# synsense/HaghighatshoarMuir2024

Measured on AMD Instinct MI355X. Metric: audio samples/sec through STHT+RZCC+SNN beamform, 7-mic 48kHz 360-DoA; DoA MAE vs ref, higher is better.
Workload: dtype f64

## Files before the change

### haghighatshoarmuir2024_amd/csrc/api.hip

```cpp
#include <math.h>
#include <string.h>

#include <new>
#include <vector>

#include "micloc_internal.h"

using namespace micloc;

static thread_local int g_last_hip = 0;

static int hip_failed(hipError_t e)
{
    g_last_hip = (int)e;
    (void)hipGetLastError();
    return MICLOC_ERR_HIP;
}

#define HIP_TRY(expr)                                \
    do {                                             \
        hipError_t _e = (expr);                      \
        if (_e != hipSuccess) return hip_failed(_e); \
    } while (0)

// ... 65 lines not shown
{
    int ct = (C + 15) / 16;
    if (ct > 4 && ct <= 8) ct = 8;
    return ct;
}

struct FrontOffsets {
    size_t h, pre, scratch, spikes;
};

struct WsLayout : FrontOffsets {
    size_t partial, total;
};

WsLayout ws_layout(const micloc_plan *p, int B, int T)
{
    WsLayout w{};
    const size_t Ts = (size_t)micloc_padded_T(T);
    const size_t planar = align256((size_t)B * p->C * Ts * sizeof(double));
    int Gp = p->W.GT > 0 ? 16 * p->W.GT : 16;
    size_t off = 0;
    w.h = off;
    off += planar;
    w.pre = off;
    off += planar;
    w.scratch = off;
    off += rzcc_scratch_bytes(B * p->C, T, p->robust_width, p->chunk_frames);
    w.spikes = off;
    off += align256((size_t)B * T * p->C);
    w.partial = off;
    {
        const size_t pb = beamform_partial_bytes(B, T, Gp);
        const int ct = pad_ct(p->C);
        const size_t pc = ct <= 8 ? cov_partial_bytes(B, T, ct) : 0;
        off += pb > pc ? pb : pc;
    }
    w.total = off;
    return w;
}

bool bad_batch(int B) { return B < 1 || B > 65535; }

bool bad_ws(const void *ws, size_t have, size_t need)
{
    return ws == nullptr || have < need || (reinterpret_cast<uintptr_t>(ws) & 255) != 0;
}

double *ws_doubles(void *ws, size_t offset) { return reinterpret_cast<double *>(static_cast<unsigned char *>(ws) + offset); }

int gen_chunk_frames(int CT)
{
    for (int c = 256; c <= 4096; c += 256)
        if (beamform_nchunks_ct(c, CT) == 1 && beamform_nchunks_ct(c + 1, CT) == 2) return c;
    return 0;
}

int window_quantum(const micloc_plan *p)
{
    if (!p->W_is_complex) return lif_beamform_chunk_frames(p->W, p->ntab);
    if (p->W.CT == 1 && (p->W.GT & 1) == 0) return 256;
    return gen_chunk_frames(p->W.CT);
}

int window_args(int T, int window, int hop, int quantum, int B, int *nW)
{
    if (T < 1 || quantum < 1) return MICLOC_ERR_INVALID;
    if (window < 1 || hop < 1 || window % quantum != 0 || hop % quantum != 0) return MICLOC_ERR_SHAPE;
    const long long n = window_count(T, window, hop);
    if (n * (long long)B > 0x7fffffffll) return MICLOC_ERR_SHAPE;
    *nW = (int)n;
    return MICLOC_OK;
}

int window_readout(const micloc_plan *p, const double *partial, int B, int T, int nch, int quantum, int window, int hop, double *power_w,
                   int32_t *argmax_w, double *power, int32_t *argmax, hipStream_t st)
{
    if (nch != (T + quantum - 1) / quantum) return MICLOC_ERR_INVALID;
    const int Gp = 16 * p->W.GT, cp = p->W_is_complex ? 1 : 0;
    HIP_TRY(launch_window_power(partial, B, T, nch, Gp, p->G_out, cp, cp ? Gp / 2 : 0, quantum, window, hop, power_w, argmax_w, st));
    if (power || argmax) HIP_TRY(launch_power_argmax(partial, B, T, nch, Gp, p->G_out, cp, cp ? Gp / 2 : 0, power, argmax, st));
    return MICLOC_OK;
}

hipError_t lif_beamform_oneshot(const BeamformW &W, const NeuronTab &nt, const int8_t *spikes, int B, int T, double *y, double *partial,
                                hipStream_t stream, int *nchunks)
{
    hipError_t e = hipSuccess;
    if (launch_lif_beamform_lean(W, nt, spikes, B, T, y, partial, stream, nchunks, &e)) return e;
    return launch_lif_beamform(W, nt, spikes, B, T, y, partial, stream, nchunks);
}

int plan_kind(const micloc_plan *p, bool cpx)
{
    if (!p->d_W || (!cpx && !p->d_ntab)) return MICLOC_ERR_NOT_SET;
    return (p->W_is_complex != 0) == cpx ? MICLOC_OK : MICLOC_ERR_SHAPE;
}

int window_check(const micloc_plan *p, bool cpx, int B, int T, int window, int hop)
{
    int rc = plan_kind(p, cpx), nW = 0;
    if (rc != MICLOC_OK) return rc;
    const int q = window_quantum(p);
    rc = window_args(T, window, hop, q, B, &nW);
    return rc == MICLOC_OK ? q : rc;
}

int cov_check(const micloc_plan *p, bool want_power)
{
    if (!p->d_ntab) return MICLOC_ERR_NOT_SET;
    if (want_power && (!p->d_W || p->W_is_complex)) return p->d_W ? MICLOC_ERR_SHAPE : MICLOC_ERR_NOT_SET;
    return pad_ct(p->C) > 8 ? MICLOC_ERR_SHAPE : MICLOC_OK;
}

struct Front {
    int rc;
    const void *src;
    int Ts;
};

Front front_end(const micloc_plan *p, bool cpx, const double *x, int B, int T, void *ws, const FrontOffsets &o, int8_t *spikes, int stages,
                hipStream_t st)
{
    Front f{MICLOC_OK, nullptr, micloc_padded_T(T)};
    double *h = ws_doubles(ws, o.h);
    hipError_t e = (stages & MICLOC_STAGE_STHT) ? launch_stht(p->taps, x, h, B, T, p->M, f.Ts, st, false) : hipSuccess;
    if (cpx) {
        double *pre = ws_doubles(ws, o.pre);
        f.src = pre;
        if (e == hipSuccess)
            e = launch_bandpass_rzcc(p->iir, h, B * p->C, p->C, T, f.Ts, p->robust_width, p->bipolar, pre, nullptr, nullptr, st, x, p->M,
                                     p->taps.shift);
    } else {
        int8_t *spk = spikes ? spikes : static_cast<int8_t *>(ws) + o.spikes;
        f.src = spk;
        const int phases = (stages & MICLOC_STAGE_ENCODE) ? RZ_PHASE_ALL
                                                          : ((stages & MICLOC_STAGE_ENCODE_SCAN) ? RZ_PHASE_SCAN : 0) |
                                                                ((stages & MICLOC_STAGE_ENCODE_REST) ? RZ_PHASE_ENCODE : 0);
        if (e == hipSuccess && phases)
            e = launch_bandpass_rzcc(p->iir, h, B * p->C, p->C, T, f.Ts, p->robust_width, p->bipolar, nullptr, spk,
                                     static_cast<char *>(ws) + o.scratch, st, x, p->M, p->taps.shift, p->chunk_frames, phases);
    }
    if (e != hipSuccess) f.rc = hip_failed(e);
    return f;
}

int power_tail(const micloc_plan *p, const void *src, int B, int T, int Ts, double *y, double *power, int32_t *argmax, double *partial,
               hipStream_t st)
{
    const int Gp = 16 * p->W.GT, cpx = p->W_is_complex ? 1 : 0;
    if (!power && !argmax) partial = nullptr;
    int nch = 0;
    if (cpx)
        HIP_TRY(launch_planar_beamform(p->W, static_cast<const double *>(src), B, T, Ts, y, 1, partial, st, &nch));
    else
        HIP_TRY(lif_beamform_oneshot(p->W, p->ntab, static_cast<const int8_t *>(src), B, T, y, partial, st, &nch));
    if (partial) HIP_TRY(launch_power_argmax(partial, B, T, nch, Gp, p->G_out, cpx, cpx ? Gp / 2 : 0, power, argmax, st));
    return MICLOC_OK;
}

int window_tail(const micloc_plan *p, const void *src, int B, int T, int Ts, int quantum, int window, int hop, double *power_w,
                int32_t *argmax_w, double *power, int32_t *argmax, double *partial, hipStream_t st)
{
    int nch = 0;
    if (p->W_is_complex)
        HIP_TRY(launch_planar_beamform(p->W, static_cast<const double *>(src), B, T, Ts, nullptr, 1, partial, st, &nch));
    else
        HIP_TRY(launch_lif_beamform(p->W, p->ntab, static_cast<const int8_t *>(src), B, T, nullptr, partial, st, &nch));
    return window_readout(p, partial, B, T, nch, quantum, window, hop, power_w, argmax_w, power, argmax, st);
}

int cov_tail(const micloc_plan *p, const int8_t *spikes, int B, int T, int t_start, double *cov, double *power, int32_t *argmax, double *partial,
             hipStream_t st)
{
    const int CT = pad_ct(p->C);
    const bool want_power = power || argmax;
    HIP_TRY(launch_lif_cov(p->ntab, spikes, B, T, p->C, CT, t_start, partial, st));
    HIP_TRY(launch_cov_power(partial, B, T, CT, p->C, T - t_start, want_power ? p->W.Wp : nullptr, want_power ? 16 * p->W.GT : 16,
                             want_power ? p->G_out : 0, cov, power, argmax, st));
    return MICLOC_OK;
}

}

extern "C" {

int micloc_abi_version(void) { return MICLOC_ABI_VERSION; }

int micloc_last_hip_error(void) { return g_last_hip; }

const char *micloc_status_string(int status)
{
    switch (status) {
        case MICLOC_OK: return "ok";
        case MICLOC_ERR_INVALID: return "invalid argument";
        case MICLOC_ERR_SHAPE: return "shape mismatch";
        case MICLOC_ERR_WORKSPACE: return "workspace too small or misaligned (256-byte alignment required)";
        case MICLOC_ERR_NOT_SET: return "neuron kernel or beamforming matrix not set on the plan";
        case MICLOC_ERR_HIP: return "HIP runtime error (see micloc_last_hip_error)";
        case MICLOC_ERR_NO_DEVICE: return "no usable HIP device";
        default: return "unknown status";
    }
}

int micloc_padded_T(int T) { return T <= 0 ? 8 : (T + 7) & ~7; }

int micloc_plan_create(const micloc_config *cfg, micloc_plan **out)
{
    if (!cfg || !out) return MICLOC_ERR_INVALID;
    *out = nullptr;
    if (cfg->num_mic <= 0 || cfg->stht_len <= 0 || !cfg->stht_kernel) return MICLOC_ERR_INVALID;
    if (cfg->iir_len < 1 || cfg->iir_len > MICLOC_MAX_IIR || !cfg->iir_b || !cfg->iir_a) return MICLOC_ERR_INVALID;
    if (cfg->iir_a[0] == 0.0 || cfg->robust_width < 1) return MICLOC_ERR_INVALID;
    int ndev = 0;
    if (hipGetDeviceCount(&ndev) != hipSuccess || ndev <= 0 || cfg->device < 0 || cfg->device >= ndev)
        return MICLOC_ERR_NO_DEVICE;
    {
        hipDeviceProp_t prop;
        if (hipGetDeviceProperties(&prop, cfg->device) != hipSuccess || strncmp(prop.gcnArchName, "gfx950", 6) != 0)
            return MICLOC_ERR_NO_DEVICE;
    }

    micloc_plan *p = new (std::nothrow) micloc_plan();
// ... 138 lines not shown
            Wp[(size_t)(M + m) * Gp + g] = wi;
            Wp[(size_t)m * Gp + Ghp + g] = -wi;
            Wp[(size_t)(M + m) * Gp + Ghp + g] = wr;
        }
    return set_W(p, Wp, CT, Gp / 16, C, 2 * G, 1, G);
}

int micloc_plan_generation(const micloc_plan *p) { return p ? p->generation : -1; }

int micloc_stream_create_cu_range(int device, int cu_lo, int cu_hi, void **stream)
{
    if (!stream || device < 0) return MICLOC_ERR_INVALID;
    *stream = nullptr;
    DeviceGuard guard(device);
    hipDeviceProp_t prop;
    HIP_TRY(hipGetDeviceProperties(&prop, device));
    if (strncmp(prop.gcnArchName, "gfx950", 6) != 0) return MICLOC_ERR_INVALID;
    constexpr int NXCD = 8;
    const int ncu = prop.multiProcessorCount;
    if (ncu != 256) return MICLOC_ERR_INVALID;
    const int per = ncu / NXCD;
    if (cu_lo < 0 || cu_hi > per || cu_lo >= cu_hi) return MICLOC_ERR_INVALID;
    std::vector<uint32_t> mask((size_t)(ncu + 31) / 32, 0u);
    for (int c = cu_lo; c < cu_hi; ++c)
        for (int x = 0; x < NXCD; ++x) {
            const int bit = c * NXCD + x;
            mask[bit / 32] |= 1u << (bit % 32);
        }
    hipStream_t st = nullptr;
    HIP_TRY(hipExtStreamCreateWithCUMask(&st, (uint32_t)mask.size(), mask.data()));
    *stream = st;
    return MICLOC_OK;
}

int micloc_stream_destroy(void *stream)
{
    if (!stream) return MICLOC_ERR_INVALID;
    HIP_TRY(hipStreamDestroy((hipStream_t)stream));
    return MICLOC_OK;
}

int micloc_plan_set_encoder_chunk(micloc_plan *p, int chunk_frames)
{
    if (!p) return MICLOC_ERR_INVALID;
    p->chunk_frames = chunk_frames;
    return MICLOC_OK;
}

int micloc_plan_encoder_chunks(const micloc_plan *p, int B, int T)
{
    if (!p || bad_batch(B) || T < 1) return MICLOC_ERR_INVALID;
    return rzcc_chunks(B * p->C, T, p->robust_width, p->chunk_frames);
}

size_t micloc_workspace_bytes(const micloc_plan *p, int B, int T)
{
    if (!p || bad_batch(B) || T < 1) return 0;
    return ws_layout(p, B, T).total;
}

size_t micloc_lif_beamform_workspace_bytes(const micloc_plan *p, int B, int T)
{
    if (!p || bad_batch(B) || T < 1 || p->W.GT < 1) return 0;
    return align256(beamform_partial_bytes(B, T, 16 * p->W.GT));
}

int micloc_stht_f64(const micloc_plan *p, const double *x, int B, int T, double *h, int Ts, void *stream)
{
    if (!p || !x || !h || bad_batch(B) || T < 1) return MICLOC_ERR_INVALID;
    DeviceGuard guard(p->device);
    if (Ts != micloc_padded_T(T)) return MICLOC_ERR_SHAPE;
    HIP_TRY(launch_stht(p->taps, x, h, B, T, p->M, Ts, (hipStream_t)stream));
    return MICLOC_OK;
}

int micloc_bandpass_rzcc_f64(const micloc_plan *p, const double *h, int B, int T, int Ts, double *pre,
                             int8_t *spikes, void *ws, size_t ws_bytes, void *stream)
{
    if (!p || !h || bad_batch(B) || T < 1 || (!pre && !spikes)) return MICLOC_ERR_INVALID;
    DeviceGuard guard(p->device);
    if (Ts != micloc_padded_T(T)) return MICLOC_ERR_SHAPE;
    const int nl = B * p->C;
    if (spikes && bad_ws(ws, ws_bytes, rzcc_scratch_bytes(nl, T, p->robust_width, p->chunk_frames))) return MICLOC_ERR_WORKSPACE;
    HIP_TRY(launch_bandpass_rzcc(p->iir, h, nl, p->C, T, Ts, p->robust_width, p->bipolar, pre, spikes, ws,
                                 (hipStream_t)stream, nullptr, 0, 0, p->chunk_frames));
    return MICLOC_OK;
}

int micloc_lif_beamform_f64(const micloc_plan *p, const int8_t *spikes, int B, int T, double *y, double *power,
                            int32_t *argmax, void *ws, size_t ws_bytes, void *stream)
{
    if (!p || !spikes || bad_batch(B) || T < 1 || (!y && !power && !argmax)) return MICLOC_ERR_INVALID;
    DeviceGuard guard(p->device);
    const int rc = plan_kind(p, false);
    if (rc != MICLOC_OK) return rc;
    if ((power || argmax) && bad_ws(ws, ws_bytes, beamform_partial_bytes(B, T, 16 * p->W.GT))) return MICLOC_ERR_WORKSPACE;
    return power_tail(p, spikes, B, T, 0, y, power, argmax, ws_doubles(ws, 0), (hipStream_t)stream);
}

int micloc_beamform_c128_f64(const micloc_plan *p, const double *pre, int B, int T, int Ts, double *y, double *power,
                             int32_t *argmax, void *ws, size_t ws_bytes, void *stream)
{
    if (!p || !pre || bad_batch(B) || T < 1 || (!y && !power && !argmax)) return MICLOC_ERR_INVALID;
    DeviceGuard guard(p->device);
    if (Ts != micloc_padded_T(T)) return MICLOC_ERR_SHAPE;
    const int rc = plan_kind(p, true);
    if (rc != MICLOC_OK) return rc;
    if ((power || argmax) && bad_ws(ws, ws_bytes, beamform_partial_bytes(B, T, 16 * p->W.GT))) return MICLOC_ERR_WORKSPACE;
    return power_tail(p, pre, B, T, Ts, y, power, argmax, ws_doubles(ws, 0), (hipStream_t)stream);
}

int micloc_snn_pipeline_f64(const micloc_plan *p, const double *x, int B, int T, int8_t *spikes, double *y,
                            double *power, int32_t *argmax, void *ws, size_t ws_bytes, void *stream)
{
    return micloc_snn_pipeline_stages_f64(p, x, B, T, spikes, y, power, argmax, ws, ws_bytes, stream, MICLOC_STAGE_ALL);
}

int micloc_snn_pipeline_stages_f64(const micloc_plan *p, const double *x, int B, int T, int8_t *spikes, double *y,
                                   double *power, int32_t *argmax, void *ws, size_t ws_bytes, void *stream, int stages)
{
    if (!p || !x || bad_batch(B) || T < 1 || (!spikes && !y && !power && !argmax)) return MICLOC_ERR_INVALID;
    DeviceGuard guard(p->device);
    if (stages <= 0 || (stages & ~(MICLOC_STAGE_ALL | MICLOC_STAGE_ENCODE_SCAN | MICLOC_STAGE_ENCODE_REST))) return MICLOC_ERR_INVALID;
    const bool want_bf = y || power || argmax;
    const int rc = want_bf ? plan_kind(p, false) : MICLOC_OK;
    if (rc != MICLOC_OK) return rc;
    const WsLayout w = ws_layout(p, B, T);
    if (bad_ws(ws, ws_bytes, w.total)) return MICLOC_ERR_WORKSPACE;
    const Front f = front_end(p, false, x, B, T, ws, w, spikes, stages, (hipStream_t)stream);
    if (f.rc != MICLOC_OK) return f.rc;
    if (!want_bf || !(stages & MICLOC_STAGE_BEAMFORM)) return MICLOC_OK;
    return power_tail(p, f.src, B, T, f.Ts, y, power, argmax, ws_doubles(ws, w.partial), (hipStream_t)stream);
}

int micloc_beamformer_pipeline_f64(const micloc_plan *p, const double *x, int B, int T, double *y, double *power,
                                   int32_t *argmax, void *ws, size_t ws_bytes, void *stream)
{
    if (!p || !x || bad_batch(B) || T < 1 || (!y && !power && !argmax)) return MICLOC_ERR_INVALID;
    DeviceGuard guard(p->device);
    const int rc = plan_kind(p, true);
    if (rc != MICLOC_OK) return rc;
    const WsLayout w = ws_layout(p, B, T);
    if (bad_ws(ws, ws_bytes, w.total)) return MICLOC_ERR_WORKSPACE;
    const Front f = front_end(p, true, x, B, T, ws, w, nullptr, MICLOC_STAGE_ALL, (hipStream_t)stream);
    if (f.rc != MICLOC_OK) return f.rc;
    return power_tail(p, f.src, B, T, f.Ts, y, power, argmax, ws_doubles(ws, w.partial), (hipStream_t)stream);
}

int micloc_window_quantum(const micloc_plan *p)
{
    if (!p) return MICLOC_ERR_INVALID;
    if (plan_kind(p, p->W_is_complex) != MICLOC_OK) return MICLOC_ERR_NOT_SET;
    const int q = window_quantum(p);
    return q > 0 ? q : MICLOC_ERR_INVALID;
}

int micloc_window_count(int T, int window, int hop, int quantum)
{
    int nW = 0;
    const int rc = window_args(T, window, hop, quantum, 1, &nW);
    return rc == MICLOC_OK ? nW : rc;
}

size_t micloc_window_workspace_bytes(const micloc_plan *p, int B, int T, int window, int hop, int pipeline)
{
    if (!p || bad_batch(B) || T < 1 || micloc_window_quantum(p) < 1) return 0;
    int nW = 0;
    if (window_args(T, window, hop, window_quantum(p), B, &nW) != MICLOC_OK) return 0;
// ... 1219 lines not shown
```

### haghighatshoarmuir2024_amd/csrc/micloc_internal.h

```cpp
#pragma once
#include <hip/hip_runtime.h>
#include <stddef.h>
#include <stdint.h>

#include "../../include/micloc_hip.h"

namespace micloc {

constexpr bool VARIANT_WS_FOUR_KSTEPS = false;
constexpr bool VARIANT_STHT_VECTOR_FORM = false;
constexpr bool VARIANT_STHT_WIDE_TWO_TILES = false;
constexpr bool VARIANT_STHT_ONE_TILE = false;
constexpr bool VARIANT_WS_GENERAL_ONLY = false;

__device__ __forceinline__ int xcd_walk(int L, int n)
{
    const int per = n >> 3;
    return L < 8 * per ? (L & 7) * per + (L >> 3) : L;
}

constexpr int STHT_R = 8;
constexpr int STHT_TILE = 64 * STHT_R;
constexpr int STHT_MAX_MB = 8;

struct SthtTaps {
    const double *taps;
    int ngroups;
    int klo;
    int kstep;
    int halo;
    int shift;
};

hipError_t launch_stht(const SthtTaps &tp, const double *x, double *h, int B, int T, int M, int Ts,
                       hipStream_t stream, bool write_re = true);
size_t stht_lds_bytes(const SthtTaps &tp, int M);

struct IirCoef {
    double b[MICLOC_MAX_IIR];
    double a[MICLOC_MAX_IIR];
    int n;
};

size_t rzcc_scratch_bytes(int nlanes, int T, int robust_width, int chunk_frames);
int rzcc_chunks(int nlanes, int T, int robust_width, int chunk_frames);
constexpr int RZ_PHASE_SCAN = 1, RZ_PHASE_ENCODE = 2, RZ_PHASE_ALL = 3;
hipError_t launch_bandpass_rzcc(const IirCoef &coef, const double *h, int nlanes, int C, int T, int Ts,
                                int robust_width, int bipolar, double *pre, int8_t *spikes, void *scratch,
                                hipStream_t stream, const double *xin = nullptr, int M = 0, int shift = 0,
                                int chunk_frames = 0, int phases = RZ_PHASE_ALL);
size_t rzcc_stream_state_bytes(int nlanes);
hipError_t launch_stream_encode(const IirCoef &coef, const double *h, int nlanes, int C, int T, int Ts, int robust_width,
                                int bipolar, int8_t *spikes, int Ttot, long long t_base, int first_tile, int final_tile,
                                void *state, hipStream_t stream, int pos_lo = 0, const int *clk = nullptr);
hipError_t launch_stream_horizon(const void *enc_state, int nlanes, int bipolar, int t_end, int final_, int chunk_frames, int base_chunk,
                                 int nwin, int *ctl, hipStream_t stream, int clocked = 0);
constexpr int STREAM_CLK_T = 16;
constexpr int STREAM_CLK_BASE = 17;
constexpr int STREAM_CLK_SHIFT = 18;
constexpr int STREAM_CLK_TEND = 19;
hipError_t launch_stream_begin_tile(int *ctl, int8_t *win, int8_t *tmp, int B, size_t row_bytes, int C, int n, int cap, int chunk_frames,
                                    hipStream_t stream);
hipError_t launch_stream_tick(int *ctl, hipStream_t stream);
hipError_t launch_stht_wrap_rows(double *h, const double *wrap, int B, int M, int Ts, int col0, int n, int half, const int *ctl,
                                 hipStream_t stream);
hipError_t launch_stream_commit(int *ctl, int block_chunks, hipStream_t stream);
hipError_t launch_stream_accumulate(const double *partial, int B, int nwin, int Gp, int G, const int *range, const int *ctl,
                                    double *acc, const int *frames_ptr, double *power, int32_t *argmax, hipStream_t stream);
constexpr int STREAM_BLOCK_CHUNKS = 32;
hipError_t launch_zero_fill(void *ptr, size_t bytes, hipStream_t stream);
hipError_t launch_pack_planar(const double *src, double *dst, int B, int T, int C, int Ts, hipStream_t stream);
hipError_t launch_unpack_planar(const double *src, double *dst, int B, int T, int C, int Ts, hipStream_t stream);

constexpr int BF_WAVES = 8;
constexpr int BF_NT = 4;
constexpr int BF_CHUNK = BF_WAVES * BF_NT * 16;

struct BeamformW {
    const double *Wp;
    int CT, GT;
    int C, G;
    int complex_pairs;
    const int *chunk_range = nullptr;
};

struct NeuronTab {
    const double *tab;
    int n;
    int NK;
};

size_t beamform_partial_bytes(int B, int T, int Gp);
hipError_t launch_lif_beamform(const BeamformW &W, const NeuronTab &nt, const int8_t *spikes, int B, int T,
                               double *y, double *partial, hipStream_t stream, int *nchunks);
bool launch_lif_beamform_lean(const BeamformW &W, const NeuronTab &nt, const int8_t *spikes, int B, int T, double *y, double *partial,
                              hipStream_t stream, int *nchunks, hipError_t *err);
hipError_t launch_planar_beamform(const BeamformW &W, const double *pre, int B, int T, int Ts, double *y,
                                  int y_complex, double *partial, hipStream_t stream, int *nchunks);
hipError_t launch_power_argmax(const double *partial, int B, int T, int nchunks, int Gp, int G, int complex_pairs,
                               int Ghalf_pad, double *power, int32_t *argmax, hipStream_t stream);
int beamform_nchunks(int T);
int beamform_nchunks_ct(int T, int CT);
int lif_beamform_chunk_frames(const BeamformW &W, const NeuronTab &nt);

long long window_count(int T, int window, int hop);
hipError_t launch_window_power(const double *partial, int B, int T, int nchunks, int Gp, int G, int complex_pairs, int Ghalf_pad,
                               int chunk_frames, int window, int hop, double *power_w, int32_t *argmax_w, hipStream_t stream);

int stream_window_slots(int window, int hop);
size_t stream_window_state_bytes(int B, int G, int window, int hop);
hipError_t launch_stream_windows(const double *partial, int B, int nwin, int Gp, int G, int complex_pairs, int Ghp, int chunk_frames,
                                 const int *ctl, int final_tile, int window, int hop, int max_windows, void *win_state, double *power_w,
                                 int32_t *argmax_w, double *latest_power, int32_t *latest_argmax, hipStream_t stream);

struct StreamComplexLayout {
    size_t z, carry, acc, total;
};
StreamComplexLayout stream_complex_layout(int B, int C, int G, int iir_n, int CH);
int stream_complex_chunks(int max_tile, int CH);
hipError_t launch_stream_complex_bandpass(const IirCoef &co, const double *h, int nl, int n, size_t row_stride, double *staging, int S,
                                          int CH, void *state, const StreamComplexLayout &L, hipStream_t stream);
hipError_t launch_stream_complex_accumulate(const double *partial, int B, int Ks, int Gp, int G, int CH, int final_tile, void *state,
                                            const StreamComplexLayout &L, double *power, int32_t *argmax, hipStream_t stream);
hipError_t launch_stream_complex_slide(const double *staging, int nl, int S, int CH, void *state, const StreamComplexLayout &L,
                                       hipStream_t stream);

hipError_t launch_lif_beamform_f32(const BeamformW &W, const NeuronTab &nt, const int8_t *spikes, int B, int T,
                                   double *partial, hipStream_t stream, int *nchunks);

size_t cov_partial_bytes(int B, int T, int CT);
hipError_t launch_lif_cov(const NeuronTab &nt, const int8_t *spikes, int B, int T, int C, int CT, int t_start,
                          double *partial, hipStream_t stream);
hipError_t launch_cov_power(const double *partial, int B, int T, int CT, int C, int Tn, const double *Wp, int Gp, int G,
// ... 111 lines not shown
```

Before: 3.727 billion.

## Add warp-specialized single-pass RZCC sweep kernel with fallback for overflowing lanes

Adds a new bandpass+RZCC spike encoder that uses dedicated loader waves, an IIR/cumsum wave and a zero-crossing/cluster-resolve wave. They run in a triple-buffered LDS pipeline, one block per 64 lanes. Lanes whose ring overflows are flagged and reprocessed by a per-lane fallback kernel. The path is used when the filter order is 5, the encode phase is requested and a single chunk covers T; otherwise the old launcher runs. It aims to cut the multi-pass scan/encode cost but adds a zero-fill pass and a fallback launch, with complex correctness conditions.

New measurement: 3.864 billion (median of 6 runs). 3.7% higher.

```diff
diff --git a/haghighatshoarmuir2024_amd/csrc/api.hip b/haghighatshoarmuir2024_amd/csrc/api.hip
--- a/haghighatshoarmuir2024_amd/csrc/api.hip
+++ b/haghighatshoarmuir2024_amd/csrc/api.hip
@@ -171,6 +171,18 @@
     return MICLOC_OK;
 }
 
+static hipError_t bandpass_rzcc_spikes(const IirCoef &coef, const double *h, int nlanes, int C, int T, int Ts, int robust_width, int bipolar,
+                                       int8_t *spikes, void *scratch, hipStream_t stream, const double *xin, int M, int shift,
+                                       int chunk_frames, int phases)
+{
+    hipError_t e = hipSuccess;
+    if (launch_bandpass_rzcc_sweep(coef, h, nlanes, C, T, Ts, robust_width, bipolar, spikes, scratch, stream, xin, M, shift, chunk_frames,
+                                   phases, &e))
+        return e;
+    return launch_bandpass_rzcc(coef, h, nlanes, C, T, Ts, robust_width, bipolar, nullptr, spikes, scratch, stream, xin, M, shift,
+                                chunk_frames, phases);
+}
+
 hipError_t lif_beamform_oneshot(const BeamformW &W, const NeuronTab &nt, const int8_t *spikes, int B, int T, double *y, double *partial,
                                 hipStream_t stream, int *nchunks)
 {
@@ -226,7 +238,7 @@
                                                           : ((stages & MICLOC_STAGE_ENCODE_SCAN) ? RZ_PHASE_SCAN : 0) |
                                                                 ((stages & MICLOC_STAGE_ENCODE_REST) ? RZ_PHASE_ENCODE : 0);
         if (e == hipSuccess && phases)
-            e = launch_bandpass_rzcc(p->iir, h, B * p->C, p->C, T, f.Ts, p->robust_width, p->bipolar, nullptr, spk,
+            e = bandpass_rzcc_spikes(p->iir, h, B * p->C, p->C, T, f.Ts, p->robust_width, p->bipolar, spk,
                                      static_cast<char *>(ws) + o.scratch, st, x, p->M, p->taps.shift, p->chunk_frames, phases);
     }
     if (e != hipSuccess) f.rc = hip_failed(e);
@@ -531,8 +543,12 @@
     if (Ts != micloc_padded_T(T)) return MICLOC_ERR_SHAPE;
     const int nl = B * p->C;
     if (spikes && bad_ws(ws, ws_bytes, rzcc_scratch_bytes(nl, T, p->robust_width, p->chunk_frames))) return MICLOC_ERR_WORKSPACE;
-    HIP_TRY(launch_bandpass_rzcc(p->iir, h, nl, p->C, T, Ts, p->robust_width, p->bipolar, pre, spikes, ws,
-                                 (hipStream_t)stream, nullptr, 0, 0, p->chunk_frames));
+    if (spikes && !pre)
+        HIP_TRY(bandpass_rzcc_spikes(p->iir, h, nl, p->C, T, Ts, p->robust_width, p->bipolar, spikes, ws, (hipStream_t)stream, nullptr, 0, 0,
+                                     p->chunk_frames, RZ_PHASE_ALL));
+    else
+        HIP_TRY(launch_bandpass_rzcc(p->iir, h, nl, p->C, T, Ts, p->robust_width, p->bipolar, pre, spikes, ws,
+                                     (hipStream_t)stream, nullptr, 0, 0, p->chunk_frames));
     return MICLOC_OK;
 }
 
diff --git a/haghighatshoarmuir2024_amd/csrc/micloc_internal.h b/haghighatshoarmuir2024_amd/csrc/micloc_internal.h
--- a/haghighatshoarmuir2024_amd/csrc/micloc_internal.h
+++ b/haghighatshoarmuir2024_amd/csrc/micloc_internal.h
@@ -12,6 +12,7 @@
 constexpr bool VARIANT_STHT_WIDE_TWO_TILES = false;
 constexpr bool VARIANT_STHT_ONE_TILE = false;
 constexpr bool VARIANT_WS_GENERAL_ONLY = false;
+constexpr bool VARIANT_RZ_TWO_SLOTS = false;
 
 __device__ __forceinline__ int xcd_walk(int L, int n)
 {
@@ -49,6 +50,9 @@
                                 int robust_width, int bipolar, double *pre, int8_t *spikes, void *scratch,
                                 hipStream_t stream, const double *xin = nullptr, int M = 0, int shift = 0,
                                 int chunk_frames = 0, int phases = RZ_PHASE_ALL);
+bool launch_bandpass_rzcc_sweep(const IirCoef &coef, const double *h, int nlanes, int C, int T, int Ts, int robust_width, int bipolar,
+                                int8_t *spikes, void *scratch, hipStream_t stream, const double *xin, int M, int shift, int chunk_frames,
+                                int phases, hipError_t *err);
 size_t rzcc_stream_state_bytes(int nlanes);
 hipError_t launch_stream_encode(const IirCoef &coef, const double *h, int nlanes, int C, int T, int Ts, int robust_width,
                                 int bipolar, int8_t *spikes, int Ttot, long long t_base, int first_tile, int final_tile,
diff --git a/haghighatshoarmuir2024_amd/csrc/rzcc_sweep.hip b/haghighatshoarmuir2024_amd/csrc/rzcc_sweep.hip
--- /dev/null
+++ b/haghighatshoarmuir2024_amd/csrc/rzcc_sweep.hip
@@ -0,0 +1,758 @@
+#include "micloc_internal.h"
+
+#include <type_traits>
+
+#pragma clang diagnostic ignored "-Wpass-failed"
+
+namespace micloc {
+namespace rzsweep {
+
+constexpr int RZ_RING_SWEEP = 32;
+
+template <int N>
+struct Iir {
+    double z[N > 1 ? N - 1 : 1];
+
+    __device__ __forceinline__ void init()
+    {
+#pragma unroll
+        for (int i = 0; i < (N > 1 ? N - 1 : 1); ++i) z[i] = 0.0;
+    }
+
+    __device__ __forceinline__ double step(const IirCoef &coef, double xin)
+    {
+        double y;
+        if (N == 1) {
+            y = __builtin_fma(coef.b[0], xin, 0.0);
+        } else {
+            y = __builtin_fma(coef.b[0], xin, z[0]);
+#pragma unroll
+            for (int i = 0; i < N - 2; ++i)
+                z[i] = __builtin_fma(-coef.a[i + 1], y, __builtin_fma(coef.b[i + 1], xin, z[i + 1]));
+            z[N - 2] = __builtin_fma(-coef.a[N - 1], y, coef.b[N - 1] * xin);
+        }
+        return y;
+    }
+};
+
+template <int N>
+__device__ __forceinline__ void pin_coef(const IirCoef &coef)
+{
+#pragma unroll
+    for (int i = 0; i < N; ++i) asm volatile("; filter coefficient resident" ::"s"(coef.b[i]), "s"(coef.a[i]));
+}
+
+template <int W, typename WordAt, typename ValAt, typename Emit>
+__device__ __forceinline__ void resolve_cluster_regs(int s, int stride, int count, int w, Emit emit, WordAt word_at, ValAt val_at,
+                                                     double sgn)
+{
+    int P[W];
+    double V[W];
+#pragma unroll
+    for (int u = 0; u < W; ++u) {
+        const int kc = u < count ? s + u * stride : s;
+        P[u] = *word_at(kc) >> 1;
+        V[u] = *val_at(kc) * sgn;
+    }
+    unsigned alive = (1u << count) - 1u;
+    while (alive) {
+        int best = -1, pb = 0;
+        double bv = 0.0;
+#pragma unroll
+        for (int u = 0; u < W; ++u) {
+            if (((alive >> u) & 1u) && (best < 0 || V[u] >= bv)) {
+                best = u;
+                bv = V[u];
+                pb = P[u];
+            }
+        }
+        emit(pb);
+        alive &= ~(1u << best);
+#pragma unroll
+        for (int u = 0; u < W; ++u) {
+            const int d = P[u] - pb;
+            if ((d < 0 ? -d : d) < w) alive &= ~(1u << u);
+        }
+    }
+}
+
+template <int MAXW = 16, typename WordAt, typename ValAt, typename Emit>
+__device__ __forceinline__ void resolve_cluster(int s, int e, int stride, int w, Emit emit, WordAt word_at, ValAt val_at,
+                                                double sgn)
+{
+    int remaining = (e - s + stride - 1) / stride;
+    if (remaining <= 4) {
+        resolve_cluster_regs<4>(s, stride, remaining, w, emit, word_at, val_at, sgn);
+        return;
+    }
+    if (remaining <= 8) {
+        resolve_cluster_regs<8>(s, stride, remaining, w, emit, word_at, val_at, sgn);
+        return;
+    }
+    if (MAXW >= 16 && remaining <= 16) {
+        resolve_cluster_regs<16>(s, stride, remaining, w, emit, word_at, val_at, sgn);
+        return;
+    }
+    while (remaining > 0) {
+        int best = -1;
+        double bv = 0.0;
+        for (int k = s; k < e; k += 4 * stride) {
+            int wk[4];
+            double vk[4];
+#pragma unroll
+            for (int u = 0; u < 4; ++u) {
+                const int kk = k + u * stride;
+                const int kc = kk < e ? kk : s;
+                wk[u] = *word_at(kc);
+                vk[u] = *val_at(kc) * sgn;
+            }
+#pragma unroll
+            for (int u = 0; u < 4; ++u) {
+                const int kk = k + u * stride;
+                if (kk < e && wk[u] >= 0 && (best < 0 || vk[u] >= bv)) {
+                    best = kk;
+                    bv = vk[u];
+                }
+            }
+        }
+        const int wb = *word_at(best);
+        const int pb = wb >> 1;
+        emit(pb);
+        *word_at(best) = ~wb;
+        --remaining;
+        for (int k = best - stride; k >= s; k -= stride) {
+            const int wk = *word_at(k);
+            const int pk = (wk < 0 ? ~wk : wk) >> 1;
+            if (pb - pk >= w) break;
+            if (wk >= 0) {
+                *word_at(k) = ~wk;
+                --remaining;
+            }
+        }
+        for (int k = best + stride; k < e; k += stride) {
+            const int wk = *word_at(k);
+            const int pk = (wk < 0 ? ~wk : wk) >> 1;
+            if (pk - pb >= w) break;
+            if (wk >= 0) {
+                *word_at(k) = ~wk;
+                --remaining;
+            }
+        }
+    }
+}
+
+constexpr int RZ_MT = 16;
+
+__device__ __forceinline__ void rise_fall_step(unsigned &r, unsigned &f, double a, double b)
+{
+    asm("v_cmp_gt_f64 vcc, %2, %3\n\tv_addc_co_u32_e32 %0, vcc, %0, %0, vcc\n\tv_cmp_lt_f64 vcc, %2, %3\n\tv_addc_co_u32_e32 %1, vcc, %1, %1, vcc"
+        : "+v"(r), "+v"(f)
+        : "v"(a), "v"(b)
+        : "vcc");
+}
+
+struct RzGeom {
+    int P;
+    int Lt;
+    int Vt;
+    int V2t;
+};
+
+struct RzSpan {
+    int m_lo, m_hi;
+    int own_lo, own_hi;
+    bool at_end;
+};
+
+__host__ __device__ inline RzSpan rz_span(const RzGeom &g, int p, int NM)
+{
+    RzSpan s;
+    s.m_lo = p == 0 ? 0 : p * g.Lt - g.Vt;
+    const int hi = (p + 1) * g.Lt + g.V2t;
+    s.m_hi = (p == g.P - 1 || hi > NM) ? NM : hi;
+    s.own_lo = p == 0 ? 0 : p * g.Lt * RZ_MT;
+    s.own_hi = p == g.P - 1 ? 0x7fffffff : (p + 1) * g.Lt * RZ_MT;
+    s.at_end = s.m_hi == NM;
+    return s;
+}
+
+constexpr int RZ_DIR_RISE = 1, RZ_DIR_FALL = 2, RZ_DIR_UNKNOWN = 3;
+
+template <int PHASE, typename XT>
+__device__ __forceinline__ void rz_loader_np(XT &X, const double *__restrict__ h, const double *__restrict__ xin, int base,
+                                             int nlanes, int C, int T, int Ts, int M, int shift, int NMc, int nstep, int lane,
+                                             unsigned long long *tab)
+{
+    constexpr int NP = 2;
+    constexpr int phase = PHASE;
+    const int tl = lane & 15;
+    const int sq = lane >> 4;
+    constexpr int NJ = 16;
+    double v[2][NJ];
+    {
+        int g = base + lane;
+        g = g < nlanes ? g : nlanes - 1;
+        const int bb = g / C, cc = g - bb * C;
+        const bool r = xin != nullptr && cc < M;
+        const double *b0 = r ? xin + (size_t)bb * T * M + cc : h + (size_t)g * Ts;
+        tab[lane] = (unsigned long long)(size_t)b0 | (r ? 1ull : 0ull);
+        __builtin_amdgcn_fence(__ATOMIC_RELEASE, "wavefront");
+        __builtin_amdgcn_wave_barrier();
+        __builtin_amdgcn_fence(__ATOMIC_ACQUIRE, "wavefront");
+    }
+    const int sh = shift % T;
+    auto issue_loads = [&](int q, auto set) {
+        constexpr int S = decltype(set)::value;
+        int mm = phase + NP * q;
+        mm = mm < NMc ? mm : NMc - 1;
+        const int t = mm * RZ_MT + tl;
+        const int tc = t < Ts ? t : Ts - 1;
+        int tr = (t < T ? t : T - 1) - sh;
+        tr = tr < 0 ? tr + T : tr;
+        const unsigned i_roll = (unsigned)tr * (unsigned)M, i_lin = (unsigned)tc;
+        {
+            const unsigned ta = (unsigned)(size_t)(&tab[sq]);
+            typedef __attribute__((address_space(1))) double gdouble;
+#pragma unroll
+            for (int j0 = 0; j0 < NJ; j0 += 4) {
+                unsigned long long e[4];
+#pragma unroll
+                for (int u = 0; u < 4; ++u)
+                    asm volatile("ds_read_b64 %0, %1 offset:%2" : "=v"(e[u]) : "v"(ta), "n"((j0 + u) * 32));
+                asm volatile("s_waitcnt lgkmcnt(0)" : "+v"(e[0]), "+v"(e[1]), "+v"(e[2]), "+v"(e[3]));
+#pragma unroll
+                for (int u = 0; u < 4; ++u)
+                    v[S][j0 + u] = reinterpret_cast<const gdouble *>((size_t)(e[u] & ~7ull))[(e[u] & 1ull) ? i_roll : i_lin];
+            }
+        }
+    };
+    auto write_tile = [&](int buf, auto set) {
+        constexpr int S = decltype(set)::value;
+        {
+            const unsigned wa = (unsigned)(size_t)(&X[buf][tl][sq]);
+#pragma unroll
+            for (int j = 0; j < NJ; ++j) {
+                const double vj = v[S][j];
+                asm volatile("ds_write_b64 %0, %1 offset:%2" ::"v"(wa), "v"(vj), "n"(j * 32));
+            }
+        }
+    };
+    using set0 = std::integral_constant<int, 0>;
+    using set1 = std::integral_constant<int, 1>;
+    issue_loads(0, set0{});
+    issue_loads(1, set1{});
+    if (phase == 0) {
+        write_tile(0, set0{});
+        issue_loads(2, set0{});
+    }
+    __syncthreads();
+    auto iter = [&](int k, auto pos, auto set) {
+        constexpr int I = decltype(pos)::value;
+        if constexpr (((I + 1) % NP) == phase) {
+            const int m = k + 1;
+            write_tile(m % 3, set);
+            issue_loads((m - phase) / NP + 2, set);
+        }
+        __syncthreads();
+    };
+    using p0 = std::integral_constant<int, 0>;
+    using p1 = std::integral_constant<int, 1>;
+    using p2 = std::integral_constant<int, 2>;
+    using p3 = std::integral_constant<int, 3>;
+    int k = 0;
+    for (; k + 3 < nstep; k += 4) {
+        iter(k, p0{}, set0{});
+        iter(k + 1, p1{}, set1{});
+        iter(k + 2, p2{}, set1{});
+        iter(k + 3, p3{}, set0{});
+    }
+    if (k < nstep) iter(k++, p0{}, set0{});
+    if (k < nstep) iter(k++, p1{}, set1{});
+    if (k < nstep) iter(k++, p2{}, set1{});
+}
+
+template <int N, int RING>
+__global__ __launch_bounds__(384, 5) void bandpass_rzcc_sweep_kernel(const double *__restrict__ h, int8_t *__restrict__ spikes,
+                                                                     int *__restrict__ flag_count, int *__restrict__ flag_list,
+                                                                     IirCoef coef, int nlanes, int C, int T, int Ts, int w, int bipolar,
+                                                                     const double *__restrict__ xin, int M, int shift)
+{
+    constexpr int SW = 64;
+    constexpr int ROW = SW + 1;
+    __shared__ __attribute__((aligned(16))) double X[3][RZ_MT][ROW];
+    __shared__ double ringV[RING][SW];
+    __shared__ int ringP[RING][SW];
+    __shared__ int nPub[SW];
+    __shared__ int polPub[SW];
+    __shared__ int deadPub[SW];
+    __shared__ int ovPub[SW];
+    __shared__ int oldPub[2][SW];
+    __shared__ unsigned long long ldTab[SW];
+
+    const int wave_hw = threadIdx.x >> 6;
+    const int wave = wave_hw == 0 ? 0 : wave_hw - 1;
+    const int lane = threadIdx.x & 63;
+    const int base = xcd_walk(blockIdx.x, gridDim.x) * SW;
+    const int NM = (T + RZ_MT - 1) / RZ_MT;
+    const int NSTEP = NM + 2;
+    const int lane_g = base + lane;
+    const bool active = lane_g < nlanes;
+    const int lane_c = active ? lane_g : nlanes - 1;
+
+    if (wave_hw == 0) {
+        rz_loader_np<0>(X, h, xin, base, nlanes, C, T, Ts, M, shift, NM, NSTEP, lane, ldTab);
+        return;
+    }
+    if (wave_hw == 1) {
+        rz_loader_np<1>(X, h, xin, base, nlanes, C, T, Ts, M, shift, NM, NSTEP, lane, ldTab);
+        return;
+    }
+
+    if (wave == 1) {
+        Iir<N> iir;
+        iir.init();
+        double cs = 0.0;
+        pin_coef<N>(coef);
+        __syncthreads();
+        for (int k = 0; k < NSTEP; ++k) {
+            if (k < NM) {
+                const int buf = k % 3;
+                const int tb = k * RZ_MT;
+                const int steps = (T - tb) < RZ_MT ? (T - tb) : RZ_MT;
+                if (steps == RZ_MT) {
+                    double xr[RZ_MT];
+                    const unsigned addr = (unsigned)(size_t)(&X[buf][0][lane]);
+#pragma unroll
+                    for (int j = 0; j < RZ_MT; ++j)
+                        asm volatile("ds_read_b64 %0, %1 offset:%2" : "=v"(xr[j]) : "v"(addr), "n"(j * ROW * 8));
+                    asm volatile("s_waitcnt lgkmcnt(0)"
+                                 : "+v"(xr[0]), "+v"(xr[1]), "+v"(xr[2]), "+v"(xr[3]), "+v"(xr[4]), "+v"(xr[5]), "+v"(xr[6]), "+v"(xr[7]),
+                                   "+v"(xr[8]), "+v"(xr[9]), "+v"(xr[10]), "+v"(xr[11]), "+v"(xr[12]), "+v"(xr[13]), "+v"(xr[14]),
+                                   "+v"(xr[15]));
+#pragma unroll
+                    for (int j = 0; j < RZ_MT; ++j) {
+                        cs = cs + iir.step(coef, xr[j]);
+                        xr[j] = cs;
+                    }
+#pragma unroll
+                    for (int j = 0; j < RZ_MT; ++j) X[buf][j][lane] = xr[j];
+                } else {
+                    for (int j = 0; j < steps; ++j) {
+                        cs = cs + iir.step(coef, X[buf][j][lane]);
+                        X[buf][j][lane] = cs;
+                    }
+                }
+            }
+            __syncthreads();
+        }
+        return;
+    }
+
+    if (wave == 2) {
+        double prev = __builtin_nan("");
+        int left = 0;
+        int n = 0;
+        int dir = 0;
+        int ffall = 0;
+        bool livel = true;
+        nPub[lane] = 0;
+        polPub[lane] = 0;
+        ovPub[lane] = 0;
+        __syncthreads();
+        for (int k = 0; k < NSTEP; ++k) {
+            if (k >= 1 && k <= NM) {
+                const int m = k - 1;
+                const int tbase = m * RZ_MT;
+                const int steps = (T - tbase) < RZ_MT ? (T - tbase) : RZ_MT;
+                const int o0 = oldPub[0][lane], o1 = oldPub[1][lane];
+                const int oldest = bipolar ? (o0 < o1 ? o0 : o1) : o0;
+                double c[RZ_MT];
+#pragma unroll
+                for (int jj = 0; jj < RZ_MT; ++jj) c[jj] = X[m % 3][jj][lane];
+                unsigned Rw = 0, Fw = 0;
+#pragma unroll
+                for (int jj = RZ_MT - 1; jj >= 0; --jj) {
+                    const double pj = jj ? c[jj ? jj - 1 : 0] : prev;
+                    rise_fall_step(Rw, Fw, c[jj], pj);
+                }
+                const unsigned vmask = (1u << steps) - 1u;
+                Rw &= vmask;
+                Fw &= vmask;
+                const unsigned Sw = Rw | Fw;
+                const unsigned Aw = (Rw | ~Sw) & 0xFFFFu;
+                const unsigned Dw = (Aw + Rw + (dir == 1 ? 1u : 0u)) ^ Aw ^ Rw;
+                const unsigned low = Sw & (0u - Sw);
+                const unsigned Hw = dir != 0 ? 0xFFFFu : (Sw ? (~(low | (low - 1u)) & 0xFFFFu) : 0u);
+                unsigned Ew = (Fw & Dw) | (bipolar ? (Rw & ~Dw & Hw) : 0u);
+                constexpr int DET_PF = 3;
+                {
+                    const int ne = __builtin_popcount(Ew);
+                    if (livel && n + (ne > DET_PF ? ne : DET_PF) - oldest > RING) {
+                        livel = false;
+                        ovPub[lane] = 1;
+                    }
+                }
+                Ew = livel ? Ew : 0u;
+                if (dir == 0 && Sw) ffall = (Fw & low) ? 1 : 0;
+                {
+                    int jev[DET_PF], lfv[DET_PF];
+                    double vev[DET_PF];
+                    const char *xt = reinterpret_cast<const char *>(&X[m % 3][0][lane]);
+#pragma unroll
+                    for (int u = 0; u < DET_PF; ++u) {
+                        const bool has = Ew != 0u;
+                        const int je = has ? __builtin_ctz(Ew) : 0;
+                        Ew &= Ew - 1u;
+                        const unsigned below = Sw & ((1u << je) - 1u);
+                        lfv[u] = below ? tbase + (31 - __builtin_clz(below)) : left;
+                        jev[u] = has ? je : -1;
+                        const double v = *reinterpret_cast<const double *>(xt + (size_t)(je > 0 ? je - 1 : 0) * ROW * 8);
+                        vev[u] = je > 0 ? v : prev;
+                    }
+                    if (livel) {
+#pragma unroll
+                        for (int u = 0; u < DET_PF; ++u) {
+                            const int slot = n & (RING - 1);
+                            ringP[slot][lane] = lfv[u] + tbase + jev[u] - 1;
+                            ringV[slot][lane] = vev[u];
+                            n += jev[u] >= 0 ? 1 : 0;
+                        }
+                    }
+                }
+                while (__any(Ew != 0u)) {
+                    if (Ew) {
+                        const int je = __builtin_ctz(Ew);
+                        Ew &= Ew - 1u;
+                        const unsigned below = Sw & ((1u << je) - 1u);
+                        const int lf = below ? tbase + (31 - __builtin_clz(below)) : left;
+                        const double val = je ? *reinterpret_cast<const double *>(reinterpret_cast<const char *>(&X[m % 3][0][lane]) +
+                                                                                 (size_t)(je - 1) * ROW * 8)
+                                              : prev;
+                        const int slot = n & (RING - 1);
+                        ringP[slot][lane] = lf + tbase + je - 1;
+                        ringV[slot][lane] = val;
+                        ++n;
+                    }
+                }
+                if (Sw) {
+                    left = tbase + (31 - __builtin_clz(Sw));
+                    dir = (Dw >> RZ_MT) & 1u ? 1 : 2;
+                }
+                prev = steps == RZ_MT ? c[RZ_MT - 1] : X[m % 3][steps - 1][lane];
+                nPub[lane] = n;
+                polPub[lane] = ffall;
+            }
+            __syncthreads();
+        }
+        return;
+    }
+
+    const int mypol = wave - 3;
+    const bool mine = bipolar || mypol == 0;
+    const int stride = bipolar ? 2 : 1;
+    int i_next = -1;
+    int s_open = -1;
+    int l_last = 0;
+    int s_first = 0;
+    bool dead = !active;
+    const int b = lane_c / C;
+    const int ch = lane_c - b * C;
+    int8_t *sp = spikes + (size_t)b * T * C + ch;
+    const int8_t mark = mypol ? -1 : 1;
+    const double sgn = mypol ? -1.0 : 1.0;
+    auto word_at = [&](int i) { return &ringP[i & (RING - 1)][lane]; };
+    auto val_at = [&](int i) { return &ringV[i & (RING - 1)][lane]; };
+    auto emit = [&](int pos) { sp[(size_t)pos * C] = mark; };
+    auto close_cluster = [&](int s, int e, int lastpos, int first) {
+        if (e - s <= stride) {
+            emit(lastpos);
+        } else if (e - s <= 2 * stride) {
+            const double v0 = *val_at(s) * sgn, v1 = *val_at(s + stride) * sgn;
+            emit(v1 >= v0 ? lastpos : first);
+        } else if (e - s <= 3 * stride) {
+            const double v0 = *val_at(s) * sgn, v1 = *val_at(s + stride) * sgn, v2 = *val_at(s + 2 * stride) * sgn;
+            const bool mid = v1 >= v0 && v2 < v1;
+            if (mid) {
+                emit(*word_at(s + stride) >> 1);
+            } else {
+                const bool last_best = v2 >= (v1 >= v0 ? v1 : v0);
+                emit(last_best ? lastpos : first);
+                if (lastpos - first >= w) emit(last_best ? first : lastpos);
+            }
+        } else {
+            resolve_cluster<8>(s, e, stride, w, emit, word_at, val_at, sgn);
+        }
+    };
+    if (mypol == 0) deadPub[lane] = 0;
+    oldPub[mypol][lane] = 0;
+    if (!mine) oldPub[mypol][lane] = 0x7fffffff;
+    __syncthreads();
+    for (int k = 0; k < NSTEP; ++k) {
+        if (k >= 2 && mine) {
+            const int n = nPub[lane];
+            if (ovPub[lane]) dead = true;
+            if (i_next < 0 && n > 0) i_next = bipolar ? (polPub[lane] ^ mypol) : 0;
+            while (__any(!dead && i_next >= 0 && i_next < n)) {
+                if (!dead && i_next >= 0 && i_next < n) {
+                    const int i = i_next;
+                    const int pos = *word_at(i) >> 1;
+                    if (s_open >= 0 && pos - l_last >= w) {
+                        close_cluster(s_open, i, l_last, s_first);
+                        s_open = -1;
+                    }
+                    if (s_open < 0) {
+                        s_open = i;
+                        s_first = pos;
+                    }
+                    l_last = pos;
+                    i_next = i + stride;
+                }
+            }
+            oldPub[mypol][lane] = dead ? 0x7fffffff : (s_open >= 0 ? s_open : (i_next >= 0 ? i_next : 0));
+        }
+        __syncthreads();
+    }
+    if (active && mine) {
+        if (ovPub[lane]) dead = true;
+        if (!dead && s_open >= 0) close_cluster(s_open, nPub[lane], l_last, s_first);
+        if (dead && atomicExch(&deadPub[lane], 1) == 0) {
+            const int kk = atomicAdd(flag_count, 1);
+            flag_list[kk] = lane_g;
+        }
+    }
+}
+
+template <int N>
+__global__ __launch_bounds__(64) void rzcc_unit_fallback_kernel(const double *__restrict__ h, int8_t *__restrict__ spikes,
+                                                                 const int *__restrict__ flag_count,
+                                                                 const int *__restrict__ flag_list, int *__restrict__ plist,
+                                                                 double *__restrict__ vlist, int nslots, IirCoef coef,
+                                                                 int nlanes, int C, int T, int Ts, int w, int bipolar,
+                                                                 const double *__restrict__ xin, int M, int shift, RzGeom g,
+                                                                 const double *__restrict__ ckd, const int *__restrict__ cki)
+{
+    const int slot = blockIdx.x * 64 + threadIdx.x;
+    if (slot >= nslots) return;
+    const int count = *flag_count;
+    const int NMall = (T + RZ_MT - 1) / RZ_MT;
+    const size_t NS = (size_t)nslots;
+    const size_t nl = (size_t)nlanes;
+    int *P = plist + slot;
+    double *V = vlist + slot;
+    const int sh = shift % T;
+    auto word_at = [&](int i) { return P + (size_t)i * NS; };
+    auto val_at = [&](int i) { return V + (size_t)i * NS; };
+
+    for (int idx = slot; idx < count; idx += nslots) {
+        const int unit = flag_list[idx];
+        const int p = unit / nlanes;
+        const int lane_g = unit - p * nlanes;
+        const RzSpan span = rz_span(g, p, NMall);
+        const int b = lane_g / C;
+        const int ch = lane_g - b * C;
+        const bool rolled = xin != nullptr && ch < M;
+        const double *src = rolled ? xin + (size_t)b * T * M + ch : h + (size_t)lane_g * Ts;
+        auto sample = [&](int t) {
+            int tr = t - sh;
+            tr = tr < 0 ? tr + T : tr;
+            return rolled ? src[(size_t)tr * M] : src[t];
+        };
+        Iir<N> iir;
+        auto load_ck = [&](int q, double &cs) {
+            iir.init();
+            cs = 0.0;
+            if (q >= 0) {
+#pragma unroll
+                for (int i = 0; i < N - 1; ++i) iir.z[i] = ckd[((size_t)q * N + i) * nl + lane_g];
+                cs = ckd[((size_t)q * N + (N - 1)) * nl + lane_g];
+            }
+        };
+        double c = 0.0;
+        int left = 0, dir = 0;
+        if (p > 0) {
+            const int dcode = cki[((size_t)(p - 1) * 3 + 0) * nl + lane_g];
+            left = cki[((size_t)(p - 1) * 3 + 1) * nl + lane_g];
+            dir = dcode == RZ_DIR_RISE ? 1 : (dcode == RZ_DIR_FALL ? -1 : 0);
+            if (dcode == RZ_DIR_UNKNOWN) {
+                const int Lc = cki[((size_t)(p - 1) * 3 + 2) * nl + lane_g];
+                int pq = (Lc + g.Vt) / g.Lt;
+                pq = pq > p - 1 ? p - 1 : pq;
+                load_ck(pq - 1, c);
+                const int t0 = pq == 0 ? 0 : (pq * g.Lt - g.Vt) * RZ_MT;
+                for (int t = t0; t < (Lc + 1) * RZ_MT; ++t) {
+                    const double c1 = c + iir.step(coef, sample(t));
+                    if (t == 0) {
+                    } else if (c1 > c) {
+                        dir = 1;
+                        left = t;
+                    } else if (c1 < c) {
+                        dir = -1;
+                        left = t;
+                    }
+                    c = c1;
+                }
+            }
+        }
+        load_ck(p - 1, c);
+        double prev = p > 0 ? c : __builtin_nan("");
+
+        int n = 0;
+        int lastpos[2] = {0, 0};
+        bool seen[2] = {false, false};
+        bool done[2] = {false, !bipolar};
+        const int t_lo = span.m_lo * RZ_MT;
+        auto walk = [&](int t, double xt) {
+            const double y = iir.step(coef, xt);
+            c = c + y;
+            const bool rise = c > prev;
+            const bool fall = c < prev;
+            if ((fall && dir > 0) || (bipolar && rise && dir < 0)) {
+                const int pol = rise ? 1 : 0;
+                const int pos = (left + t - 1) >> 1;
+                P[(size_t)n * NS] = ((left + t - 1) & ~1) | pol;
+                V[(size_t)n * NS] = rise ? -prev : prev;
+                ++n;
+                if ((!seen[pol] || pos - lastpos[pol] >= w) && pos >= span.own_hi) done[pol] = true;
+                seen[pol] = true;
+                lastpos[pol] = pos;
+            }
+            left = (rise || fall) ? t : left;
+            dir = rise ? 1 : (fall ? -1 : dir);
+            prev = c;
+            const int nextpos = dir == 0 ? t + 1 : (left + t) >> 1;
+            if (nextpos >= span.own_hi) {
+                if (!seen[0] || nextpos - lastpos[0] >= w) done[0] = true;
+                if (!seen[1] || nextpos - lastpos[1] >= w) done[1] = true;
+            }
+        };
+        constexpr int FB_BLK = 16;
+        for (int t0 = t_lo; t0 < T && !(done[0] && done[1]); t0 += FB_BLK) {
+            double xs[FB_BLK];
+#pragma unroll
+            for (int u = 0; u < FB_BLK; ++u) xs[u] = sample(t0 + u < T ? t0 + u : T - 1);
+#pragma unroll
+            for (int u = 0; u < FB_BLK; ++u)
+                if (t0 + u < T && !(done[0] && done[1])) walk(t0 + u, xs[u]);
+        }
+
+        int8_t *sp = spikes + (size_t)b * T * C + ch;
+        const int stride = bipolar ? 2 : 1;
+        const int first_pol = n > 0 ? (P[0] & 1) : 0;
+        for (int pol = 0; pol < (bipolar ? 2 : 1); ++pol) {
+            const int8_t mark = pol ? -1 : 1;
+            const int i0 = bipolar ? (first_pol == pol ? 0 : 1) : 0;
+            if (i0 >= n) continue;
+            int s = i0;
+            int plast = *word_at(i0) >> 1;
+            for (int i = i0 + stride;; i += stride) {
+                const bool has = i < n;
+                int pi = 0;
+                bool closes = true;
+                if (has) {
+                    pi = *word_at(i) >> 1;
+                    closes = (pi - plast) >= w;
+                }
+                if (closes) {
+                    const int e = has ? i : n;
+                    const int first = *word_at(s) >> 1;
+                    if (first >= span.own_lo && first < span.own_hi) {
+                        if (e - s <= stride)
+                            sp[(size_t)plast * C] = mark;
+                        else
+                            resolve_cluster(s, e, stride, w, [&](int pos) { sp[(size_t)pos * C] = mark; }, word_at, val_at, 1.0);
+                    }
+                    s = i;
+                }
+                if (!has) break;
+                plast = pi;
+            }
+        }
+    }
+}
+
+__global__ __launch_bounds__(256) void zero_fill_kernel(uint4 *__restrict__ p16, size_t n16, unsigned char *__restrict__ tail,
+                                                         int ntail, uint4 *__restrict__ extra)
+{
+    const size_t stride = (size_t)gridDim.x * 256;
+    for (size_t i = (size_t)blockIdx.x * 256 + threadIdx.x; i < n16; i += stride) p16[i] = make_uint4(0, 0, 0, 0);
+    if (blockIdx.x == 0 && (int)threadIdx.x < ntail) tail[threadIdx.x] = 0;
+    if (extra && blockIdx.x == gridDim.x - 1 && threadIdx.x < 16) extra[threadIdx.x] = make_uint4(0, 0, 0, 0);
+}
+
+static hipError_t zero_fill(void *ptr, size_t bytes, hipStream_t stream, void *extra256 = nullptr)
+{
+    const size_t n16 = bytes / 16;
+    const int ntail = (int)(bytes - n16 * 16);
+    size_t blocks = (n16 + 255) / 256;
+    if (blocks > 2048) blocks = 2048;
+    if (blocks == 0) blocks = 1;
+    hipLaunchKernelGGL(zero_fill_kernel, dim3((unsigned)blocks), dim3(256), 0, stream, reinterpret_cast<uint4 *>(ptr), n16,
+                       reinterpret_cast<unsigned char *>(ptr) + n16 * 16, ntail, reinterpret_cast<uint4 *>(extra256));
+    return hipGetLastError();
+}
+
+struct RzScratch {
+    size_t count, list, ckd, cki, vlist, plist, total;
+    int nslots;
+};
+
+static RzScratch rz_scratch(int nlanes, int T, int P)
+{
+    RzScratch s;
+    auto al = [](size_t v) { return (v + 255) & ~(size_t)255; };
+    size_t off = 0;
+    s.count = off;
+    off += 256;
+    s.list = off;
+    off += al((size_t)P * nlanes * sizeof(int));
+    s.ckd = off;
+    off += al((size_t)(P > 1 ? P - 1 : 0) * MICLOC_MAX_IIR * nlanes * sizeof(double));
+    s.cki = off;
+    off += al((size_t)(P > 1 ? P - 1 : 0) * 3 * nlanes * sizeof(int));
+    long long slots = (256ll << 20) / (12ll * (T > 0 ? T : 1));
+    if (slots < 64) slots = 64;
+    if (slots > (long long)P * nlanes) slots = (long long)P * nlanes;
+    if (slots > 4096) slots = 4096;
+    s.nslots = (int)slots;
+    s.vlist = off;
+    off += al((size_t)T * s.nslots * sizeof(double));
+    s.plist = off;
+    off += al((size_t)T * s.nslots * sizeof(int));
+    s.total = al(off);
+    return s;
+}
+
+}
+
+bool launch_bandpass_rzcc_sweep(const IirCoef &coef, const double *h, int nlanes, int C, int T, int Ts, int robust_width, int bipolar,
+                                int8_t *spikes, void *scratch, hipStream_t stream, const double *xin, int M, int shift, int chunk_frames,
+                                int phases, hipError_t *err)
+{
+    using namespace rzsweep;
+    constexpr int N = 5;
+    if (VARIANT_RZ_TWO_SLOTS || coef.n != N || !spikes || !scratch || !(phases & RZ_PHASE_ENCODE)) return false;
+    if ((unsigned long long)T * (unsigned long long)(M > 0 ? M : 1) > 0xffffffffull) return false;
+    if (rzcc_chunks(nlanes, T, robust_width, chunk_frames) != 1) return false;
+    RzGeom g;
+    g.P = 1;
+    g.Lt = (T + RZ_MT - 1) / RZ_MT;
+    g.Vt = (robust_width + RZ_MT - 1) / RZ_MT < 1 ? 1 : (robust_width + RZ_MT - 1) / RZ_MT;
+    g.V2t = 4;
+    const RzScratch sc = rz_scratch(nlanes, T, 1);
+    if (sc.total != rzcc_scratch_bytes(nlanes, T, robust_width, chunk_frames)) return false;
+    unsigned char *base = reinterpret_cast<unsigned char *>(scratch);
+    int *flag_count = reinterpret_cast<int *>(base + sc.count);
+    int *flag_list = reinterpret_cast<int *>(base + sc.list);
+    *err = zero_fill(spikes, (size_t)nlanes * T, stream, base + sc.count);
+    if (*err != hipSuccess) return true;
+    const int nblk = (nlanes + 63) / 64;
+    hipLaunchKernelGGL((bandpass_rzcc_sweep_kernel<N, RZ_RING_SWEEP>), dim3(nblk), dim3(384), 0, stream, h, spikes, flag_count, flag_list,
+                       coef, nlanes, C, T, Ts, robust_width, bipolar, xin, M, shift);
+    hipLaunchKernelGGL((rzcc_unit_fallback_kernel<N>), dim3((sc.nslots + 63) / 64), dim3(64), 0, stream, h, spikes, flag_count, flag_list,
+                       reinterpret_cast<int *>(base + sc.plist), reinterpret_cast<double *>(base + sc.vlist), sc.nslots, coef, nlanes, C, T,
+                       Ts, robust_width, bipolar, xin, M, shift, g, nullptr, nullptr);
+    *err = hipGetLastError();
+    return true;
+}
+
+}
```
